# keya-dialog/LoCo-ASR

Hardware: AMD Instinct MI355X
Metric: audio frames/sec SpeechT5-base encoder, 30s×bs32 @1/2/4/8 GPU; embed L2 vs HF (higher is better)
Workload: dtype f16x3 (fp16 hi+lo operands, 3 MFMAs per product, fp32 accumulate); 1 GPU; SpeechT5-base speech encoder, synthetic 16 kHz 30 s clips, batch 32 per GPU (BASELINE.json configs[1]), random-init weights; batch_per_gpu=32, global_batch=32, frames_per_clip=1499, parallelism=dp1, collective=none

## Files before the change

### loco-asr_amd/csrc/attention_f16x3.hip

```cpp
#include <cstdlib>

#include "loco_kernels.h"

namespace loco {

typedef _Float16 h8 __attribute__((ext_vector_type(8)));
typedef float f32x2 __attribute__((ext_vector_type(2)));
typedef unsigned u32x4 __attribute__((ext_vector_type(4)));
typedef _Float16 h4 __attribute__((ext_vector_type(4)));

constexpr int AX_BQ = 128, AX_BK = 64;
constexpr int AX_PL = AX_BK * kHeadDim;
constexpr int AX_STG = 2 * AX_PL;

typedef __attribute__((address_space(1))) const void* ax_gptr_t;
typedef __attribute__((address_space(3))) void* ax_lptr_t;

#ifndef LOCO_ATTN_HACK
#define LOCO_ATTN_HACK 0
#endif
#define AX_MFMA(a, b, c) __builtin_amdgcn_mfma_f32_32x32x16_f16(a, b, c, 0, 0, 0)
#define AX_PIN() __builtin_amdgcn_sched_barrier(0)

#ifdef LOCO_ATTN_STAMPS
__device__ unsigned long long* g_attn_stamps = nullptr;
#define AX_STAMP(k_)                                                                                                     \
    {                                                                                                                    \
        unsigned long long t_;                                                                                           \
        __builtin_amdgcn_sched_barrier(0);                                                                               \
        asm volatile("s_memtime %0\n\ts_waitcnt lgkmcnt(0)" : "=s"(t_) :: "memory");                                     \
        __builtin_amdgcn_sched_barrier(0);                                                                               \
        seg[k_] += t_ - tlast;                                                                                           \
        tlast = t_;                                                                                                      \
    }
#else
#define AX_STAMP(k_) {}
#endif

__device__ __forceinline__ void ax_split_pair(const f32x2 pv, unsigned& hi, unsigned& lo) {
    asm("s_nop 0\n\tv_cvt_pk_f16_f32 %0, %1, %2" : "=v"(hi) : "v"(pv.x), "v"(pv.y));
    asm("v_fma_mixlo_f16 %0, %1, 1.0, -%2 op_sel_hi:[0,0,1]" : "=v"(lo) : "v"(pv.x), "v"(hi));
    asm("v_fma_mixhi_f16 %0, %1, 1.0, -%2 op_sel:[0,0,1] op_sel_hi:[0,0,1]" : "+v"(lo) : "v"(pv.y), "v"(hi));
}

#ifdef LOCO_ATTN_DEBUG
__device__ float* g_attn_dbg = nullptr;
#define AX_DBG(tile_, code_, S0_, S1_)                                                                                   \
    if (g_attn_dbg && (tile_) < 8) {                                                                                     \
        float* d_ = g_attn_dbg + (((long)blockIdx.x * 256 + tid) * 8 + (tile_)) * 8;                                     \
        unsigned mask_ = 0;                                                                                              \
        float smax_ = -INFINITY, smin_ = INFINITY;                                                                       \
        _Pragma("unroll") for (int e = 0; e < 16; ++e) {                                                                 \
            if (!(fabsf(S0_[e]) <= 3e38f) && S0_[e] != -INFINITY) mask_ |= 1u;                                           \
            if (!(fabsf(S1_[e]) <= 3e38f) && S1_[e] != -INFINITY) mask_ |= 1u;                                           \
            smax_ = fmaxf(smax_, fmaxf(S0_[e], S1_[e])); smin_ = fminf(smin_, fminf(S0_[e], S1_[e]));                    \
            if (!(fabsf(o0[e]) <= 3e38f) || !(fabsf(o1[e]) <= 3e38f)) mask_ |= 2u;                                       \
        }                                                                                                                \
        if (!(fabsf(l_run) <= 3e38f)) mask_ |= 4u;                                                                       \
        if (!(fabsf(alpha) <= 3e38f)) mask_ |= 8u;                                                                       \
        if (!(fabsf(dsh) <= 3e38f)) mask_ |= 16u;                                                                        \
        d_[0] = __uint_as_float(mask_ | ((code_) << 16)); d_[1] = m_run; d_[2] = alpha; d_[3] = dsh; d_[4] = l_run;      \
        d_[5] = smax_; d_[6] = smin_; d_[7] = o0[0];                                                                     \
    }
#else
#define AX_DBG(tile_, code_, S0_, S1_) {}
#endif

typedef __fp16 ax_tr4_t __attribute__((__vector_size__(4 * sizeof(__fp16))));
__device__ __forceinline__ h8 ax_join_tr(ax_tr4_t a, ax_tr4_t b) {
    const h4 x = __builtin_bit_cast(h4, a), y = __builtin_bit_cast(h4, b);
    return h8{x[0], x[1], x[2], x[3], y[0], y[1], y[2], y[3]};
}

template <bool OUT_SPLIT, bool TABLE, bool LONG_SEQ>
__global__ __launch_bounds__(256, 2) void attention_f16x3_kernel(const _Float16* __restrict__ qhi, const _Float16* __restrict__ qlo,
                                                                 const _Float16* __restrict__ khi, const _Float16* __restrict__ klo,
                                                                 const _Float16* __restrict__ vhi, const _Float16* __restrict__ vlo,
                                                                 float* qp, const int32_t* __restrict__ frames,
                                                                 _Float16* __restrict__ ctx_hi, _Float16* __restrict__ ctx_lo,
                                                                 float* __restrict__ ctx, int T, int nqb,
                                                                 const _Float16* __restrict__ pe_hi, const _Float16* __restrict__ pe_lo,
                                                                 float pe_scale) {
    __shared__ __attribute__((aligned(16))) _Float16 lds[4 * AX_STG];
    __shared__ __attribute__((aligned(16))) float bias_stage[4][32 * 17];

    int qblk, head, b;
    {
        const int nblk = gridDim.x;
        const int q8 = nblk >> 3, r8 = nblk & 7;
        const int xcd = blockIdx.x & 7, idx = blockIdx.x >> 3;
        const int w = (xcd < r8 ? xcd * (q8 + 1) : r8 * (q8 + 1) + (xcd - r8) * q8) + idx;
        qblk = w - (w / nqb) * nqb;
        const int rest = w / nqb;
        head = rest - (rest / kHeads) * kHeads;
        b = rest / kHeads;
    }
    const int tid = threadIdx.x, lane = tid & 63;
    const int wave = __builtin_amdgcn_readfirstlane(tid >> 6);
    const int r = lane & 31, h = lane >> 5;
    const int iw0 = qblk * AX_BQ + wave * 32;
    const int iq = iw0 + r;
    const int iqc = iq < T ? iq : T - 1;

    int nvalid = frames ? frames[b] : T;
    if (nvalid <= 0 || nvalid > T) nvalid = T;
    const int ntiles = (nvalid + AX_BK - 1) / AX_BK;
    constexpr float kLog2e = 1.4426950408889634f;

    h8 qh[4], ql[4];
    {
        const long qo = ((long)b * T + iqc) * kHidden + head * kHeadDim + 8 * h;
#pragma unroll
        for (int ks = 0; ks < 4; ++ks) {
            qh[ks] = *reinterpret_cast<const h8*>(qhi + qo + 16 * ks);
            ql[ks] = *reinterpret_cast<const h8*>(qlo + qo + 16 * ks);
        }
    }
    float* qprow = qp + (((long)b * kHeads + head) * T + iqc) * kRelN;

    const int drow = lane >> 3, dpos = lane & 7;
    const unsigned lds0 = (unsigned)(unsigned long)(ax_lptr_t)lds;
    unsigned kvc[2], vvc;
#pragma unroll
    for (int i = 0; i < 2; ++i) {
        const int swz = (((2 * wave + i) & 3) << 1) | ((drow >> 1) & 1);
        kvc[i] = 2u * (unsigned)(head * kHeadDim + 8 * (dpos ^ swz));
    }
    vvc = 2u * (unsigned)(head * kHeadDim + 8 * (dpos ^ (((drow >> 1) & 1) << 2)));
    const char* const kbase_h = reinterpret_cast<const char*>(khi + (long)b * T * kHidden);
    const char* const kbase_l = reinterpret_cast<const char*>(klo + (long)b * T * kHidden);
    const char* const vbase_h = reinterpret_cast<const char*>(vhi + (long)b * T * kHidden);
    const char* const vbase_l = reinterpret_cast<const char*>(vlo + (long)b * T * kHidden);
#define AX_DMA16(base_, voff_, ldsb_) \
    asm volatile("s_mov_b32 m0, %0\n\ts_nop 0\n\tglobal_load_lds_dwordx4 %1, %2" :: "s"(ldsb_), "v"(voff_), "s"(base_) : "memory")
#define AX_DMA_PIECE(pc_, tk_, tv_, kslot_, vslot_)                                                                          \
    {                                                                                                                        \
        const int i_ = ((pc_) >> 1) & 1, pl_ = (pc_) & 1;                                                                    \
        const bool isk_ = (pc_) < 4;                                                                                         \
        const int tt_ = isk_ ? (tk_) : (tv_);                                                                                \
        const int rmax_ = T - 1 - tt_ * AX_BK;           \
        int row_ = 8 * (2 * wave + i_) + drow;                                                                               \
        row_ = row_ < rmax_ ? row_ : rmax_;                                                                                  \
        const unsigned vo_ = (unsigned)row_ * (2u * kHidden) + (isk_ ? kvc[i_] : vvc);                                       \
        const unsigned d_ = lds0 + 2u * (unsigned)((isk_ ? (kslot_) : 2 + (vslot_)) * AX_STG + pl_ * AX_PL + 8 * (2 * wave + i_) * kHeadDim); \
        AX_DMA16((isk_ ? (pl_ ? kbase_l : kbase_h) : (pl_ ? vbase_l : vbase_h)) + (long)tt_ * (AX_BK * kHidden * 2), vo_, d_); \
    }

    int fo[4];
    {
        const int swz = (((r >> 3) & 3) << 1) | ((r >> 1) & 1);
#pragma unroll
        for (int y = 0; y < 4; ++y) fo[y] = r * kHeadDim + 8 * ((2 * y + h) ^ swz);
    }
#define AX_KF(kb_, st_, ks_, pl_) (*reinterpret_cast<const h8*>((kb_) + (pl_) * AX_PL + (st_) * 32 * kHeadDim + fo[ks_]))
    int vfo[2];
    {
        const int q = (lane >> 2) & 3, pp = lane & 3, g = (lane >> 4) & 1;
#pragma unroll
        for (int dt = 0; dt < 2; ++dt)
            vfo[dt] = (4 * h + q) * kHeadDim + 8 * ((4 * (dt ^ ((q >> 1) & 1))) + 2 * g + (pp >> 1)) + 4 * (pp & 1);
    }
    typedef __fp16 ax_tr4 __attribute__((__vector_size__(4 * sizeof(__fp16))));
    typedef __attribute__((address_space(3))) ax_tr4* ax_tr4_lptr;
#define AX_VTR(vb_, dt_, c_, u_, pl_) \
    __builtin_amdgcn_ds_read_tr16_b64_v4f16((ax_tr4_lptr)((vb_) + (pl_) * AX_PL + (16 * (c_) + 8 * (u_)) * kHeadDim + vfo[dt_]))
#define AX_VF(vb_, dt_, c_, pl_) ax_join_tr(AX_VTR(vb_, dt_, c_, 0, pl_), AX_VTR(vb_, dt_, c_, 1, pl_))

    f32x16 o0, o1;
#pragma unroll
    for (int e = 0; e < 16; ++e) { o0[e] = 0.f; o1[e] = 0.f; }
    float m_run = -INFINITY, l_run = 0.f;
    float alpha = 0.f, dsh = 0.f;

    float bandv[2][2][8];
#define AX_IS_BAND(tt_) (iw0 - ((tt_) * AX_BK + AX_BK - 1) < kRelMax - 1 && iw0 + 31 - (tt_) * AX_BK > -kRelMax)
#define AX_BAND_LOAD(tt_)                                                                                              \
    if (AX_IS_BAND(tt_)) {                                                                                             \
        const float* qpb = qp + ((long)b * kHeads + head) * T * kRelN;                                                 \
        const int lj = lane & 15, lq = lane >> 4;                                                                      \
        _Pragma("unroll") for (int st_ = 0; st_ < 2; ++st_)                                                            \
            _Pragma("unroll") for (int half = 0; half < 2; ++half) {                                                   \
                const int j = (tt_) * AX_BK + 32 * st_ + 16 * half + lj;                                               \
                _Pragma("unroll") for (int u = 0; u < 8; ++u) {                                                        \
                    const int i = iw0 + 4 * u + lq;                                                                    \
                    int rel = i - j;                                                                                   \
                    rel = rel < -kRelMax ? -kRelMax : (rel > kRelMax - 1 ? kRelMax - 1 : rel);                         \
                    bandv[st_][half][u] = qpb[(long)(i < T ? i : T - 1) * kRelN + rel + kRelMax];                      \
                }                                                                                                      \
            }                                                                                                          \
    }
#define AX_BAND_ADD(S_, st_)                                                                                           \
    _Pragma("unroll") for (int half = 0; half < 2; ++half) {                                                           \
        _Pragma("unroll") for (int u = 0; u < 8; ++u) sc[66 * u + band_wr] = bandv[st_][half][u];                      \
        __builtin_amdgcn_wave_barrier();                                                                               \
        _Pragma("unroll") for (int e8 = 0; e8 < 8; ++e8)                                                               \
            S_[8 * half + e8] += sc[band_rd + (e8 & 3) + 8 * (e8 >> 2)];                                               \
        __builtin_amdgcn_wave_barrier();                                                                               \
    }
#define AX_FINISH_TILE(S0_, S1_, tt_, mx_)                                                                             \
    {                                                                                                                  \
        const int j0 = (tt_) * AX_BK;                                                                                  \
        const int dmin = iw0 - (j0 + AX_BK - 1);                                                                       \
        const int dmax = iw0 + 31 - j0;                                                                                \
        float cb = 0.f;                                                                                                \
        bool redo = false;                                                                                             \
        if (dmin >= kRelMax - 1) {                                                                                     \
            cb = c_past;                                                                                               \
        } else if (dmax <= -kRelMax) {                                                                                 \
            cb = c_future;                                                                                             \
        } else {                                                                                                       \
            float* sc = bias_stage[wave];                                                                              \
            const int lj = lane & 15, lq = lane >> 4;                                                                  \
            const int band_wr = 16 * lq + (lq >> 1) + lj, band_rd = 16 * r + (r >> 1) + 4 * h;                         \
            AX_BAND_ADD(S0_, 0)                                                                                        \
            AX_BAND_ADD(S1_, 1)                                                                                        \
            redo = true;                                                                                               \
        }                                                                                                              \
        if (j0 + AX_BK > nvalid) {                                                                                     \
            _Pragma("unroll") for (int e = 0; e < 16; ++e) {                                                           \
                const int j = j0 + (e & 3) + 8 * (e >> 2) + 4 * h;                                                     \
                S0_[e] = j < nvalid ? S0_[e] : -INFINITY;                                                              \
                S1_[e] = j + 32 < nvalid ? S1_[e] : -INFINITY;                                                         \
            }                                                                                                          \
            redo = true;                                                                                               \
        }                                                                                                              \
        float mxv = (mx_);                                                                                             \
        if (redo) {                                                                                                    \
            mxv = S0_[0];                                                                                              \
            _Pragma("unroll") for (int e = 1; e < 16; ++e) mxv = fmaxf(mxv, S0_[e]);                                   \
            _Pragma("unroll") for (int e = 0; e < 16; ++e) mxv = fmaxf(mxv, S1_[e]);                                   \
        }                                                                                                              \
        {                                               \
            float ma_ = mxv, mb_ = mxv;                                                                                \
            asm volatile("s_nop 1\n\tv_permlane32_swap_b32 %0, %1\n\ts_nop 1" : "+v"(ma_), "+v"(mb_));                \
            mxv = fmaxf(ma_, mb_) + cb;                                                                                \
        }                                                                                                              \
        const float m_new = fmaxf(m_run, mxv);                                                                         \
        alpha = __builtin_amdgcn_exp2f((m_run - m_new) * kLog2e);                                                      \
        m_run = m_new;                                                                                                 \
        dsh = (cb - m_new) * kLog2e;                                                                                   \
    }

#ifdef LOCO_ATTN_STAMPS
    unsigned long long seg[6] = {0, 0, 0, 0, 0, 0}, tlast, tstart;
    asm volatile("s_memtime %0\n\ts_waitcnt lgkmcnt(0)" : "=s"(tstart) :: "memory");
    tlast = tstart;
#endif
#pragma unroll
    for (int pc = 0; pc < 8; ++pc) AX_DMA_PIECE(pc, 0, 0, 0, 0)
    float c_past, c_future;
    if (TABLE) {
        int bmin, bmax;
        {
            int lo = iw0 - (ntiles * AX_BK - 1), hi = iw0 + 31;
            lo = lo < -kRelMax ? -kRelMax : lo;
            hi = hi > kRelMax - 1 ? kRelMax - 1 : hi;
            bmin = (lo + kRelMax) >> 5;
            bmax = (hi + kRelMax) >> 5;
        }
        float cf = 0.f, cp = 0.f;
        unsigned pev[2];
#pragma unroll
        for (int i = 0; i < 2; ++i) {
            const int swz = (((2 * wave + i) & 3) << 1) | ((drow >> 1) & 1);
            pev[i] = (unsigned)(8 * (2 * wave + i) + drow) * (2u * kHeadDim) + 16u * (unsigned)(dpos ^ swz);
        }
        const unsigned bs0 = (unsigned)(unsigned long)(ax_lptr_t)&bias_stage[0][0];
        const unsigned pev1 = (unsigned)(8 * wave + drow) * (2u * kHeadDim) + 16u * (unsigned)(dpos ^ (((wave & 3) << 1) | ((drow >> 1) & 1)));
        constexpr int kBsPlane = 32 * kHeadDim;
#define AX_PE_DMA2(b0_, slot_)                                                                                                     \
    _Pragma("unroll") for (int pc_ = 0; pc_ < 4; ++pc_) {                                                                          \
        const int i_ = (pc_ >> 1) & 1, pl_ = pc_ & 1;                                                                              \
        const unsigned d_ = lds0 + 2u * (unsigned)((slot_) * AX_STG + pl_ * AX_PL + 8 * (2 * wave + i_) * kHeadDim);               \
        AX_DMA16(reinterpret_cast<const char*>(pl_ ? pe_lo : pe_hi) + (long)(b0_) * (32 * kHeadDim * 2), pev[i_], d_);             \
    }
#define AX_PE_DMA1(b0_)                                                                                                            \
    _Pragma("unroll") for (int pl_ = 0; pl_ < 2; ++pl_) {                                                                          \
        const unsigned d_ = bs0 + 2u * (unsigned)(pl_ * kBsPlane + 8 * wave * kHeadDim);                                           \
        AX_DMA16(reinterpret_cast<const char*>(pl_ ? pe_lo : pe_hi) + (long)(b0_) * (32 * kHeadDim * 2), pev1, d_);                \
    }
        constexpr int kBlocksPerRound = kRelN / 64;
        static_assert(2 * kBlocksPerRound * 32 == kRelN && sizeof(bias_stage) >= 2 * kBsPlane * sizeof(_Float16), "table rounds");
#define AX_PE_ROUND_DMA(rd_)                                                                      \
    AX_PE_DMA2(LOCO_ATTN_HACK == 1 ? 0 : kBlocksPerRound * (rd_), 1)                               \
    AX_PE_DMA2(LOCO_ATTN_HACK == 1 ? 0 : kBlocksPerRound * (rd_) + 2, 3)                           \
    AX_PE_DMA1(LOCO_ATTN_HACK == 1 ? 0 : kBlocksPerRound * (rd_) + 4)
        AX_PE_ROUND_DMA(0)
#pragma unroll
        for (int rd = 0; rd < 2; ++rd) {
            asm volatile("s_waitcnt vmcnt(0)" ::: "memory");
            __syncthreads();
            f32x16 acc[kBlocksPerRound];
#pragma unroll
            for (int bb = 0; bb < kBlocksPerRound; ++bb) {
                const _Float16* pb = bb == 4 ? reinterpret_cast<const _Float16*>(&bias_stage[0][0]) : lds + ((bb >> 1) ? 3 : 1) * AX_STG;
                const int plane = bb == 4 ? kBsPlane : AX_PL;
#pragma unroll
                for (int e = 0; e < 16; ++e) acc[bb][e] = 0.f;
                const int blk_ = kBlocksPerRound * rd + bb;
                if (blk_ < bmin || blk_ > bmax) continue;
#pragma unroll
                for (int ks = 0; ks < 4; ++ks) {
                    const h8 fh = *reinterpret_cast<const h8*>(pb + (bb & 1) * 32 * kHeadDim + fo[ks]);
                    const h8 fl = *reinterpret_cast<const h8*>(pb + plane + (bb & 1) * 32 * kHeadDim + fo[ks]);
                    acc[bb] = AX_MFMA(fl, qh[ks], acc[bb]);
                    acc[bb] = AX_MFMA(fh, ql[ks], acc[bb]);
                    acc[bb] = AX_MFMA(fh, qh[ks], acc[bb]);
                }
            }
            __syncthreads();
            if (rd == 0) {
                AX_PE_ROUND_DMA(1)
            } else {
                const int t1 = ntiles > 1 ? 1 : 0;
#pragma unroll
                for (int pc = 0; pc < 4; ++pc) AX_DMA_PIECE(pc, t1, 0, 1, 0)
            }
#pragma unroll
            for (int bb = 0; bb < kBlocksPerRound; ++bb) {
                const int blk = kBlocksPerRound * rd + bb;
#pragma unroll
                for (int e = 0; e < 16; ++e) acc[bb][e] *= pe_scale;
                if (blk == 0) cf = acc[bb][0];
                if (blk == kRelN / 32 - 1) cp = acc[bb][15];
                if (iq < T && blk >= bmin && blk <= bmax && (LOCO_ATTN_HACK != 2 || T < 0)) {
#pragma unroll
                    for (int g4 = 0; g4 < 4; ++g4)
                        *reinterpret_cast<float4*>(qprow + 32 * blk + 8 * g4 + 4 * h) =
                            make_float4(acc[bb][4 * g4], acc[bb][4 * g4 + 1], acc[bb][4 * g4 + 2], acc[bb][4 * g4 + 3]);
                }
            }
        }
#undef AX_PE_ROUND_DMA
#undef AX_PE_DMA2
#undef AX_PE_DMA1
        float cf2 = cf, cp2 = cp;
        asm volatile("s_nop 1\n\tv_permlane32_swap_b32 %0, %1\n\ts_nop 1" : "+v"(cf), "+v"(cf2));
        asm volatile("s_nop 1\n\tv_permlane32_swap_b32 %0, %1\n\ts_nop 1" : "+v"(cp2), "+v"(cp));
        c_future = cf;
        c_past = cp;
    } else {
        const int t1 = ntiles > 1 ? 1 : 0;
#pragma unroll
        for (int pc = 0; pc < 4; ++pc) AX_DMA_PIECE(pc, t1, 0, 1, 0)
        c_past = qprow[kRelN - 1];
        c_future = qprow[0];
    }
    asm volatile("s_waitcnt vmcnt(0)" ::: "memory");
    __syncthreads();

    f32x16 sa0, sa1, sb0, sb1;
    {
#pragma unroll
        for (int e = 0; e < 16; ++e) { sa0[e] = 0.f; sa1[e] = 0.f; }
        const _Float16* kb = lds;
#pragma unroll
        for (int ks = 0; ks < 4; ++ks) {
            const h8 kh0 = AX_KF(kb, 0, ks, 0), kl0 = AX_KF(kb, 0, ks, 1), kh1 = AX_KF(kb, 1, ks, 0), kl1 = AX_KF(kb, 1, ks, 1);
            sa0 = AX_MFMA(kl0, qh[ks], sa0); sa1 = AX_MFMA(kl1, qh[ks], sa1);
            sa0 = AX_MFMA(kh0, ql[ks], sa0); sa1 = AX_MFMA(kh1, ql[ks], sa1);
            sa0 = AX_MFMA(kh0, qh[ks], sa0); sa1 = AX_MFMA(kh1, qh[ks], sa1);
        }
        float mx = sa0[0];
#pragma unroll
        for (int e = 1; e < 16; ++e) mx = fmaxf(mx, sa0[e]);
#pragma unroll
        for (int e = 0; e < 16; ++e) mx = fmaxf(mx, sa1[e]);
        AX_BAND_LOAD(0)
        AX_FINISH_TILE(sa0, sa1, 0, mx)
    }
    __syncthreads();
    AX_STAMP(5)

#define AX_ITER(t_, SC0, SC1, SN0, SN1)                                                                                \
    {                                                                                                                  \
        const int tq = (t_);                                                                                           \
        const int tkn = tq + 2 < ntiles ? tq + 2 : ntiles - 1, tvn = tq + 1 < ntiles ? tq + 1 : ntiles - 1;             \
        if (tq + 1 < ntiles) { AX_BAND_LOAD(tq + 1) }                                                                  \
        const _Float16* kb = lds + ((tq + 1) & 1) * AX_STG;                                                            \
        const _Float16* vb = lds + (2 + (tq & 1)) * AX_STG;                                                            \
        h8 kf[2][4];                                                                 \
        kf[0][0] = AX_KF(kb, 0, 0, 0); kf[0][1] = AX_KF(kb, 0, 0, 1);                                                  \
        kf[0][2] = AX_KF(kb, 1, 0, 0); kf[0][3] = AX_KF(kb, 1, 0, 1);                                                  \
        const f32x2 al2 = {alpha, alpha}, k2 = {kLog2e, kLog2e}, d2 = {dsh, dsh};                                      \
        f32x2 ps2 = {0.f, 0.f};                                                                                        \
           \
        if (!LONG_SEQ || __builtin_amdgcn_ballot_w64(alpha != 1.0f) != 0) {                                            \
            _Pragma("unroll") for (int e = 0; e < 16; e += 2) {                                                        \
                f32x2 a_ = {o0[e], o0[e + 1]}, c_ = {o1[e], o1[e + 1]};                                                \
                a_ *= al2; c_ *= al2;                                                                                  \
                o0[e] = a_.x; o0[e + 1] = a_.y; o1[e] = c_.x; o1[e + 1] = c_.y;                                        \
            }                                                                                                          \
        }                                                                                                              \
        _Pragma("unroll") for (int e = 0; e < 16; ++e) { SN0[e] = 0.f; SN1[e] = 0.f; }                                 \
        u32x4 ph0[2], pl0[2], ph1[2], pl1[2];                                                                          \
        AX_PIN();                                                                                                      \
        AX_STAMP(0)                                                                                                    \
                                                                                                     \
        _Pragma("unroll") for (int ks = 0; ks < 4; ++ks) {                                                             \
            if (ks + 1 < 4) {                                                                                          \
                kf[(ks + 1) & 1][0] = AX_KF(kb, 0, ks + 1, 0); kf[(ks + 1) & 1][1] = AX_KF(kb, 0, ks + 1, 1);          \
                kf[(ks + 1) & 1][2] = AX_KF(kb, 1, ks + 1, 0); kf[(ks + 1) & 1][3] = AX_KF(kb, 1, ks + 1, 1);          \
            }                                                                                                          \
            _Pragma("unroll") for (int m = 0; m < 6; ++m) {                                                            \
                const int st = m & 1, wh = m >> 1;                                                                     \
                const h8 a_ = kf[ks & 1][2 * st + (wh == 0 ? 1 : 0)];                                                  \
                const h8 b_ = wh == 1 ? ql[ks] : qh[ks];                                                               \
                if (st == 0) SN0 = AX_MFMA(a_, b_, SN0); else SN1 = AX_MFMA(a_, b_, SN1);                              \
                const int n = 6 * ks + m, q_ = n / 3;                                                                  \
                if (n % 3 == 0) {                                                                                      \
                    const int e0 = 2 * q_;                                                                             \
                    const f32x2 sx = {SC0[e0], SC0[e0 + 1]};                                                           \
                    const f32x2 ax = __builtin_elementwise_fma(sx, k2, d2);                                            \
                    const f32x2 pv = {__builtin_amdgcn_exp2f(ax.x), __builtin_amdgcn_exp2f(ax.y)};                     \
                    ps2 += pv;                                                                                         \
                    asm volatile("" : "+v"(ps2));                                                                      \
                    unsigned hi_, lo_;                                                                                 \
                    ax_split_pair(pv, hi_, lo_);                                                                       \
                    ph0[q_ >> 2][q_ & 3] = hi_; pl0[q_ >> 2][q_ & 3] = lo_;                                            \
                } else if (n % 3 == 1) {                                                                               \
                    const int e0 = 2 * q_;                                                                             \
                    const f32x2 sx = {SC1[e0], SC1[e0 + 1]};                                                           \
                    const f32x2 ax = __builtin_elementwise_fma(sx, k2, d2);                                            \
                    SC1[e0] = __builtin_amdgcn_exp2f(ax.x); SC1[e0 + 1] = __builtin_amdgcn_exp2f(ax.y);                \
                }                                                                                                      \
                if (n % 3 == 1 && (LOCO_ATTN_HACK != 3 || ((n / 3) & 1) == 0)) {  \
                    AX_PIN();                                                                                          \
                    AX_DMA_PIECE(n / 3, tkn, tvn, tq & 1, (tq + 1) & 1)                                                \
                }                                                                                                      \
                AX_PIN();                                                                                              \
            }                                                                                                          \
        }                                                                                                              \
        AX_STAMP(1)                                                                                                    \
                             \
        h8 vf[2][2];                                                                             \
        vf[0][0] = AX_VF(vb, 0, 0, 0); vf[0][1] = AX_VF(vb, 0, 0, 1);                                                  \
        float mxr = -INFINITY;                                                                                         \
        _Pragma("unroll") for (int g = 0; g < 8; ++g) {                                                                \
            const int st = g >> 2, s2 = (g >> 1) & 1, dt = g & 1;                                                      \
            if (g + 1 < 8) {                                                                                           \
                const int c1 = (g + 1) >> 1, dt1 = (g + 1) & 1;                                                        \
                vf[(g + 1) & 1][0] = AX_VF(vb, dt1, c1, 0); vf[(g + 1) & 1][1] = AX_VF(vb, dt1, c1, 1);                \
            }                                                                                                          \
            const h8 vh = vf[g & 1][0], vl = vf[g & 1][1];                                                             \
            const h8 ph = __builtin_bit_cast(h8, st == 0 ? ph0[s2] : ph1[s2]);                                         \
            const h8 pl = __builtin_bit_cast(h8, st == 0 ? pl0[s2] : pl1[s2]);                                         \
            _Pragma("unroll") for (int m = 0; m < 3; ++m) {                                                            \
                const h8 a_ = m == 0 ? vl : vh;                                                                        \
                const h8 b_ = m == 1 ? pl : ph;                                                                        \
                if (dt == 0) o0 = AX_MFMA(a_, b_, o0); else o1 = AX_MFMA(a_, b_, o1);                                  \
                const int n = 3 * g + m;                                                                               \
                if (n < 8) {                          \
                    const f32x2 pv = {SC1[2 * n], SC1[2 * n + 1]};                                                     \
                    ps2 += pv;                                                                                         \
                    asm volatile("" : "+v"(ps2));                                                                      \
                    unsigned hi_, lo_;                                                                                 \
                    ax_split_pair(pv, hi_, lo_);                                                                       \
                    ph1[n >> 2][n & 3] = hi_; pl1[n >> 2][n & 3] = lo_;                                                \
                } else if (n >= 12 && n < 20) {              \
                    const int e0 = 4 * (n - 12);                                                                       \
                    if (e0 < 16) mxr = fmaxf(fmaxf(fmaxf(mxr, SN0[e0]), fmaxf(SN0[e0 + 1], SN0[e0 + 2])), SN0[e0 + 3]); \
                    else mxr = fmaxf(fmaxf(fmaxf(mxr, SN1[e0 - 16]), fmaxf(SN1[e0 - 15], SN1[e0 - 14])), SN1[e0 - 13]); \
                    asm volatile("" : "+v"(mxr));                                                                      \
                }                                                                                                      \
                AX_PIN();                                                                                              \
            }                                                                                                          \
        }                                                                                                              \
        l_run = l_run * alpha + (ps2.x + ps2.y);                                                                       \
        AX_STAMP(2)                                                                                                    \
        if (tq + 1 < ntiles) { AX_FINISH_TILE(SN0, SN1, tq + 1, mxr) }                                                 \
        AX_DBG(tq, 1u, SN0, SN1)                                                                                       \
        AX_STAMP(3)                                                                                                    \
        asm volatile("s_waitcnt vmcnt(0)" ::: "memory");                                                               \
        __syncthreads();                                                                                               \
        AX_STAMP(4)                                                                                                    \
    }

    for (int t = 0; t < ntiles; t += 2) {
        AX_ITER(t, sa0, sa1, sb0, sb1)
        if (t + 1 >= ntiles) break;
        AX_ITER(t + 1, sb0, sb1, sa0, sa1)
    }
#undef AX_ITER
#undef AX_FINISH_TILE
#undef AX_BAND_LOAD
#undef AX_BAND_ADD
#undef AX_IS_BAND
#undef AX_DMA_PIECE
#undef AX_DMA16
#undef AX_KF
#undef AX_VF
#undef AX_VTR

#ifdef LOCO_ATTN_STAMPS
    if (g_attn_stamps && tid == 0) {
        unsigned long long* o_ = g_attn_stamps + 8l * blockIdx.x;
        for (int k_ = 0; k_ < 6; ++k_) o_[k_] = seg[k_];
        o_[6] = (unsigned long long)ntiles;
        o_[7] = tlast - tstart;
    }
#endif
    const float l_tot = l_run + __shfl_xor(l_run, 32, 64);
    const float inv = 1.0f / l_tot;
    if (iq < T) {
        const long obase = ((long)b * T + iq) * kHidden + head * kHeadDim + 4 * h;
#pragma unroll
        for (int g4 = 0; g4 < 4; ++g4) {
            float a[4], c[4];
#pragma unroll
            for (int e = 0; e < 4; ++e) {
                a[e] = o0[4 * g4 + e] * inv;
                c[e] = o1[4 * g4 + e] * inv;
            }
            if (OUT_SPLIT) {
                typedef unsigned u32x2 __attribute__((ext_vector_type(2)));
                unsigned h0, l0, h1, l1;
                split_f16_2pairs(a[0], a[1], a[2], a[3], h0, l0, h1, l1);
                *reinterpret_cast<u32x2*>(ctx_hi + obase + 8 * g4) = u32x2{h0, h1};
                *reinterpret_cast<u32x2*>(ctx_lo + obase + 8 * g4) = u32x2{l0, l1};
                split_f16_2pairs(c[0], c[1], c[2], c[3], h0, l0, h1, l1);
                *reinterpret_cast<u32x2*>(ctx_hi + obase + 32 + 8 * g4) = u32x2{h0, h1};
                *reinterpret_cast<u32x2*>(ctx_lo + obase + 32 + 8 * g4) = u32x2{l0, l1};
            } else {
                *reinterpret_cast<float4*>(ctx + obase + 8 * g4) = make_float4(a[0], a[1], a[2], a[3]);
                *reinterpret_cast<float4*>(ctx + obase + 32 + 8 * g4) = make_float4(c[0], c[1], c[2], c[3]);
            }
        }
    }
}

static int read_attn_long_knob() {
    const char* v = getenv("LOCO_ATTN_LONG");
    return v ? (atoi(v) != 0) : -1;
}
static int& attn_long_knob() {
    static int k = read_attn_long_knob();
    return k;
}
void reload_attention_knobs() { attn_long_knob() = read_attn_long_knob(); }

hipError_t launch_attention_f16x3(const _Float16* qhi, const _Float16* qlo, const _Float16* khi, const _Float16* klo,
                                  const _Float16* vhi, const _Float16* vlo, const float* qp, const int32_t* frames,
                                  _Float16* ctx_hi, _Float16* ctx_lo, float* ctx, int B, int T, hipStream_t s,
                                  const _Float16* pe_hi, const _Float16* pe_lo, float pe_scale) {
    if (B <= 0 || T <= 0 || B > 65535) return hipErrorInvalidValue;
    const int nqb = (T + AX_BQ - 1) / AX_BQ;
    const long nblk = (long)nqb * kHeads * B;
    if (nblk > 0x7fffffffL) return hipErrorInvalidValue;
    dim3 grid((unsigned)nblk);
    float* qpw = const_cast<float*>(qp);
    if ((pe_hi == nullptr) != (pe_lo == nullptr)) return hipErrorInvalidValue;
    const int forced = attn_long_knob();
    const bool long_seq = forced < 0 ? T >= 4096 : forced != 0;
#define AX_LAUNCH1(SPLIT_, TABLE_, LONG_)                                                                                              \
    hipLaunchKernelGGL((attention_f16x3_kernel<SPLIT_, TABLE_, LONG_>), grid, dim3(256), 0, s, qhi, qlo, khi, klo, vhi, vlo, qpw, frames, ctx_hi, \
                       ctx_lo, ctx, T, nqb, pe_hi, pe_lo, pe_scale)
#define AX_LAUNCH(SPLIT_, TABLE_)                    \
    {                                                \
        if (long_seq) AX_LAUNCH1(SPLIT_, TABLE_, true); \
        else AX_LAUNCH1(SPLIT_, TABLE_, false);      \
    }
    if (ctx_hi && pe_hi) AX_LAUNCH(true, true)
    else if (ctx_hi) AX_LAUNCH(true, false)
    else if (pe_hi) AX_LAUNCH(false, true)
    else AX_LAUNCH(false, false)
#undef AX_LAUNCH
#undef AX_LAUNCH1
    return hipGetLastError();
}

}

#ifdef LOCO_ATTN_DEBUG
extern "C" int loco_debug_set_attn_dbg(void* buf) {
    return (int)hipMemcpyToSymbol(HIP_SYMBOL(loco::g_attn_dbg), &buf, sizeof(buf));
}
#endif
#ifdef LOCO_ATTN_STAMPS
extern "C" int loco_debug_set_attn_stamps(void* buf) {
    return (int)hipMemcpyToSymbol(HIP_SYMBOL(loco::g_attn_stamps), &buf, sizeof(buf));
}
#endif
```

Measured before the change: 934,200 frames/s.

## Transpose rel-pos bias tile through LDS for coalesced stores; restage table in three rounds

```diff
diff --git a/loco-asr_amd/csrc/attention_f16x3.hip b/loco-asr_amd/csrc/attention_f16x3.hip
--- a/loco-asr_amd/csrc/attention_f16x3.hip
+++ b/loco-asr_amd/csrc/attention_f16x3.hip
@@ -265,36 +265,31 @@
             const int swz = (((2 * wave + i) & 3) << 1) | ((drow >> 1) & 1);
             pev[i] = (unsigned)(8 * (2 * wave + i) + drow) * (2u * kHeadDim) + 16u * (unsigned)(dpos ^ swz);
         }
-        const unsigned bs0 = (unsigned)(unsigned long)(ax_lptr_t)&bias_stage[0][0];
-        const unsigned pev1 = (unsigned)(8 * wave + drow) * (2u * kHeadDim) + 16u * (unsigned)(dpos ^ (((wave & 3) << 1) | ((drow >> 1) & 1)));
-        constexpr int kBsPlane = 32 * kHeadDim;
 #define AX_PE_DMA2(b0_, slot_)                                                                                                     \
     _Pragma("unroll") for (int pc_ = 0; pc_ < 4; ++pc_) {                                                                          \
         const int i_ = (pc_ >> 1) & 1, pl_ = pc_ & 1;                                                                              \
         const unsigned d_ = lds0 + 2u * (unsigned)((slot_) * AX_STG + pl_ * AX_PL + 8 * (2 * wave + i_) * kHeadDim);               \
-        AX_DMA16(reinterpret_cast<const char*>(pl_ ? pe_lo : pe_hi) + (long)(b0_) * (32 * kHeadDim * 2), pev[i_], d_);             \
-    }
-#define AX_PE_DMA1(b0_)                                                                                                            \
-    _Pragma("unroll") for (int pl_ = 0; pl_ < 2; ++pl_) {                                                                          \
-        const unsigned d_ = bs0 + 2u * (unsigned)(pl_ * kBsPlane + 8 * wave * kHeadDim);                                           \
-        AX_DMA16(reinterpret_cast<const char*>(pl_ ? pe_lo : pe_hi) + (long)(b0_) * (32 * kHeadDim * 2), pev1, d_);                \
-    }
-        constexpr int kBlocksPerRound = kRelN / 64;
-        static_assert(2 * kBlocksPerRound * 32 == kRelN && sizeof(bias_stage) >= 2 * kBsPlane * sizeof(_Float16), "table rounds");
-#define AX_PE_ROUND_DMA(rd_)                                                                      \
-    AX_PE_DMA2(LOCO_ATTN_HACK == 1 ? 0 : kBlocksPerRound * (rd_), 1)                               \
-    AX_PE_DMA2(LOCO_ATTN_HACK == 1 ? 0 : kBlocksPerRound * (rd_) + 2, 3)                           \
-    AX_PE_DMA1(LOCO_ATTN_HACK == 1 ? 0 : kBlocksPerRound * (rd_) + 4)
-        AX_PE_ROUND_DMA(0)
-#pragma unroll
-        for (int rd = 0; rd < 2; ++rd) {
+        AX_DMA16(reinterpret_cast<const char*>(pl_ ? pe_lo : pe_hi) + (long)(LOCO_ATTN_HACK == 1 ? 0 : (b0_)) * (32 * kHeadDim * 2), pev[i_], d_); \
+    }
+        constexpr int kRounds = 3, kBlocksPerRound = 4;
+        static_assert((kRounds - 1) * kBlocksPerRound + 2 == kRelN / 32, "table rounds");
+        float* const tsc = bias_stage[wave];
+        static_assert(sizeof(bias_stage[0]) >= 16 * 32 * sizeof(float), "transposition scratch: 16 queries x 128 bytes");
+        const int t_wr = 32 * (r & 15) + 4 * (h ^ (r & 7));
+        const int t_rd = 32 * (lane >> 3) + 4 * ((lane & 7) ^ (lane >> 3));
+        float* const qpw0 = qp + (((long)b * kHeads + head) * T + iw0) * kRelN + (lane >> 3) * kRelN + 4 * (lane & 7);
+        AX_PE_DMA2(0, 1)
+        AX_PE_DMA2(2, 3)
+#pragma unroll
+        for (int rd = 0; rd < kRounds; ++rd) {
+            const int nbb = rd == kRounds - 1 ? 2 : kBlocksPerRound;
             asm volatile("s_waitcnt vmcnt(0)" ::: "memory");
             __syncthreads();
             f32x16 acc[kBlocksPerRound];
 #pragma unroll
             for (int bb = 0; bb < kBlocksPerRound; ++bb) {
-                const _Float16* pb = bb == 4 ? reinterpret_cast<const _Float16*>(&bias_stage[0][0]) : lds + ((bb >> 1) ? 3 : 1) * AX_STG;
-                const int plane = bb == 4 ? kBsPlane : AX_PL;
+                if (bb >= nbb) continue;
+                const _Float16* pb = lds + ((rd == kRounds - 1 || (bb >> 1)) ? 3 : 1) * AX_STG;
 #pragma unroll
                 for (int e = 0; e < 16; ++e) acc[bb][e] = 0.f;
                 const int blk_ = kBlocksPerRound * rd + bb;
@@ -302,38 +297,61 @@
 #pragma unroll
                 for (int ks = 0; ks < 4; ++ks) {
                     const h8 fh = *reinterpret_cast<const h8*>(pb + (bb & 1) * 32 * kHeadDim + fo[ks]);
-                    const h8 fl = *reinterpret_cast<const h8*>(pb + plane + (bb & 1) * 32 * kHeadDim + fo[ks]);
+                    const h8 fl = *reinterpret_cast<const h8*>(pb + AX_PL + (bb & 1) * 32 * kHeadDim + fo[ks]);
                     acc[bb] = AX_MFMA(fl, qh[ks], acc[bb]);
                     acc[bb] = AX_MFMA(fh, ql[ks], acc[bb]);
                     acc[bb] = AX_MFMA(fh, qh[ks], acc[bb]);
                 }
             }
-            __syncthreads();
+            if (rd < kRounds - 1) __syncthreads();
             if (rd == 0) {
-                AX_PE_ROUND_DMA(1)
-            } else {
+                AX_PE_DMA2(4, 1)
+                AX_PE_DMA2(6, 3)
+            } else if (rd == 1) {
+                AX_PE_DMA2(8, 3)
                 const int t1 = ntiles > 1 ? 1 : 0;
 #pragma unroll
                 for (int pc = 0; pc < 4; ++pc) AX_DMA_PIECE(pc, t1, 0, 1, 0)
             }
 #pragma unroll
             for (int bb = 0; bb < kBlocksPerRound; ++bb) {
+                if (bb >= nbb) continue;
                 const int blk = kBlocksPerRound * rd + bb;
 #pragma unroll
                 for (int e = 0; e < 16; ++e) acc[bb][e] *= pe_scale;
                 if (blk == 0) cf = acc[bb][0];
                 if (blk == kRelN / 32 - 1) cp = acc[bb][15];
-                if (iq < T && blk >= bmin && blk <= bmax && (LOCO_ATTN_HACK != 2 || T < 0)) {
-#pragma unroll
-                    for (int g4 = 0; g4 < 4; ++g4)
-                        *reinterpret_cast<float4*>(qprow + 32 * blk + 8 * g4 + 4 * h) =
-                            make_float4(acc[bb][4 * g4], acc[bb][4 * g4 + 1], acc[bb][4 * g4 + 2], acc[bb][4 * g4 + 3]);
+                if (blk >= bmin && blk <= bmax && (LOCO_ATTN_HACK != 2 || T < 0)) {
+                    float4 tv0, tv1, tv2, tv3;
+                    if (r < 16) {
+#pragma unroll
+                        for (int g4 = 0; g4 < 4; ++g4)
+                            *reinterpret_cast<float4*>(tsc + (t_wr ^ (8 * g4))) =
+                                make_float4(acc[bb][4 * g4], acc[bb][4 * g4 + 1], acc[bb][4 * g4 + 2], acc[bb][4 * g4 + 3]);
+                    }
+                    __builtin_amdgcn_wave_barrier();
+                    tv0 = *reinterpret_cast<const float4*>(tsc + t_rd);
+                    tv1 = *reinterpret_cast<const float4*>(tsc + t_rd + 8 * 32);
+                    __builtin_amdgcn_wave_barrier();
+                    if (r >= 16) {
+#pragma unroll
+                        for (int g4 = 0; g4 < 4; ++g4)
+                            *reinterpret_cast<float4*>(tsc + (t_wr ^ (8 * g4))) =
+                                make_float4(acc[bb][4 * g4], acc[bb][4 * g4 + 1], acc[bb][4 * g4 + 2], acc[bb][4 * g4 + 3]);
+                    }
+                    __builtin_amdgcn_wave_barrier();
+                    tv2 = *reinterpret_cast<const float4*>(tsc + t_rd);
+                    tv3 = *reinterpret_cast<const float4*>(tsc + t_rd + 8 * 32);
+                    __builtin_amdgcn_wave_barrier();
+                    const int i0 = iw0 + (lane >> 3);
+                    if (i0 < T) *reinterpret_cast<float4*>(qpw0 + 32 * blk) = tv0;
+                    if (i0 + 8 < T) *reinterpret_cast<float4*>(qpw0 + 8 * kRelN + 32 * blk) = tv1;
+                    if (i0 + 16 < T) *reinterpret_cast<float4*>(qpw0 + 16 * kRelN + 32 * blk) = tv2;
+                    if (i0 + 24 < T) *reinterpret_cast<float4*>(qpw0 + 24 * kRelN + 32 * blk) = tv3;
                 }
             }
         }
-#undef AX_PE_ROUND_DMA
 #undef AX_PE_DMA2
-#undef AX_PE_DMA1
         float cf2 = cf, cp2 = cp;
         asm volatile("s_nop 1\n\tv_permlane32_swap_b32 %0, %1\n\ts_nop 1" : "+v"(cf), "+v"(cf2));
         asm volatile("s_nop 1\n\tv_permlane32_swap_b32 %0, %1\n\ts_nop 1" : "+v"(cp2), "+v"(cp));
@@ -502,7 +520,7 @@
 #endif
     const float l_tot = l_run + __shfl_xor(l_run, 32, 64);
     const float inv = 1.0f / l_tot;
-    if (iq < T) {
+    if (iq < T && (LOCO_ATTN_HACK != 4 || T < 0)) {
         const long obase = ((long)b * T + iq) * kHidden + head * kHeadDim + 4 * h;
 #pragma unroll
         for (int g4 = 0; g4 < 4; ++g4) {
```

Result: no change. 934,700 frames/s (median of 2 runs) (+0.1%).
